# jimonld2000/AudioDenoiser

Measured on AMD Instinct MI355X. Metric: spectrogram frames/sec (forward), 513x256 fp32, higher is better.
Workload: dtype f32; 1 GPU; BASELINE configs[1]: batch=64 synthetic 513x256 fp32 spectrograms on one MI355X, full U-Net forward + per-clip perceptual loss; batch_per_gpu=64, global_batch=64, freq_bins=513, frames=256, parallelism=clips sharded over 1 rank(s), weights replicated, no data-path collective, lib_digest=616623384a0f

## Files before the change

audiodenoiser_amd/csrc/adn_internal.h:

```cpp
#pragma once
#include <hip/hip_runtime.h>
#include <atomic>
#include <cstddef>
#include <cstdint>
#include <type_traits>

namespace adn {

template <typename T> constexpr int ACT_BLOCK = 32 / (int)sizeof(T);
template <typename T>
__host__ __device__ __forceinline__ long act_off(int C, long HW, long pix, int c)
{
    constexpr int B = ACT_BLOCK<T>;
    (void)C;
    return ((long)(c / B) * HW + pix) * B + (c % B);
}

#ifdef __HIPCC__
typedef float f32x2 __attribute__((ext_vector_type(2)));
typedef float f32x4 __attribute__((ext_vector_type(4)));
typedef float f32x16 __attribute__((ext_vector_type(16)));
typedef _Float16 f16x2 __attribute__((ext_vector_type(2)));
typedef _Float16 f16x4 __attribute__((ext_vector_type(4)));
typedef _Float16 f16x8 __attribute__((ext_vector_type(8)));
// ... 185 lines not shown
struct ConvGeom {
    int TH;
    int BN;
    int KC;
};
ConvGeom conv_geom(ConvKind kind, int Cout, bool f16);
long conv_mfma_tiles(ConvKind kind, bool f16, ConvArgs &a);

template <auto... KERNELS>
hipError_t lds_opt_in(size_t bytes)
{
    static std::atomic<unsigned long long> done{0};
    int dev = 0;
    if (hipGetDevice(&dev) != hipSuccess) return hipErrorInvalidDevice;
    const unsigned long long bit = 1ull << (dev & 63);
    if (done.load(std::memory_order_acquire) & bit) return hipSuccess;
    for (const void *k : {reinterpret_cast<const void *>(KERNELS)...}) {
        const hipError_t e = hipFuncSetAttribute(k, hipFuncAttributeMaxDynamicSharedMemorySize, (int)bytes);
        if (e != hipSuccess) return e;
    }
    done.fetch_or(bit, std::memory_order_release);
    return hipSuccess;
}
inline int device_cus()
{
    static std::atomic<int> cus{0};
    int c = cus.load(std::memory_order_relaxed);
    if (c == 0) {
        int dev = 0;
        if (hipGetDevice(&dev) != hipSuccess || hipDeviceGetAttribute(&c, hipDeviceAttributeMultiprocessorCount, dev) != hipSuccess || c < 8)
            return 0;
        c &= ~7;
        cus.store(c, std::memory_order_relaxed);
    }
    return c;
}

hipError_t launch_conv_mfma(ConvKind kind, const ConvArgs &a, bool f16, hipStream_t st);
hipError_t launch_conv_reduce(ConvKind kind, const ConvArgs &a, bool f16, hipStream_t st);
hipError_t launch_convt_reduce(const float *partial, const float *bias, float *out, int ksplit, int N, int Ho, int Wo, int Cout,
                               hipStream_t st);
constexpr int WINO_BN = 32;
hipError_t launch_wino_conv(ConvKind kind, const ConvArgs &a, hipStream_t st);
long wino_tiles(ConvArgs &a);
bool wino4_applicable(ConvKind kind, const ConvArgs &a, bool force);
long wino4_workgroups(const ConvArgs &a);
hipError_t launch_wino4_conv(ConvKind kind, const ConvArgs &a, hipStream_t st);

struct Wino3sGeom {
    int tilesY, tilesX;
    long rows;
    size_t v_bytes, m_bytes;
    long gemm_grid;
};
enum SplitTile { SPLIT_BN128 = 0, SPLIT_BN256 = 1, SPLIT_BN256W8 = 2 };
inline int split_tile_bn(SplitTile t) { return t == SPLIT_BN128 ? 128 : 256; }
bool wino3s_applicable(ConvKind kind, const ConvArgs &a);
Wino3sGeom wino3s_geom(const ConvArgs &a);
hipError_t launch_wino3s_conv(ConvKind kind, const ConvArgs &a, float *V, float *M, SplitTile tile, hipStream_t st);
hipError_t launch_wino_gemm(const float *V, const void *U, float *M, long rows, int Cin, int Cout, SplitTile tile, hipStream_t st);

bool conv16_applicable(ConvKind kind, const ConvArgs &a);
hipError_t launch_conv16(ConvKind kind, const ConvArgs &a, bool resident, hipStream_t st);

bool convt16_applicable(const ConvArgs &a);
hipError_t launch_convt16(const ConvArgs &a, hipStream_t st);

hipError_t launch_conv_first(const float *x, const float *w9x64, const float *bias, void *out, bool f16,
                             int N, int H, int W, int Cin, hipStream_t st);
hipError_t launch_dot_finish(const float *planes, int nplanes, float bias, float *y, long npix, hipStream_t st);
hipError_t launch_conv_out(const void *in, bool f16, const float *w64, float bias, float *out, long npix, long HW,
                           long out_stride, hipStream_t st);
hipError_t launch_nhwc_to_nchw(const void *in, bool f16, float *out, int N, int H, int W, int C, hipStream_t st);

hipError_t launch_stft_mag(const float *audio, int n_clips, long L, int n_fft, int hop, int center, long n_frames,
                           float *out, int rows, long row_stride, long clip_stride, int quantize, hipStream_t st);
constexpr hipError_t ADN_COLD_IN_CAPTURE = hipErrorStreamCaptureUnsupported;
bool stream_is_capturing(hipStream_t st);
hipError_t stft_tables(int n_fft, const float **out, hipStream_t st);
hipError_t loss_tables(hipStream_t st);
hipError_t launch_gl_polar(const float *mag, const float *rnd, int n_clips, int F, int T, void *spec, hipStream_t st);
hipError_t launch_istft_frames(const void *spec, int n_clips, int T, int n_fft, float *buf, hipStream_t st);
hipError_t launch_istft_ola(const float *buf, int n_clips, int T, int n_fft, int hop, float *audio, hipStream_t st);
hipError_t launch_stft_complex(const float *audio, int n_clips, long L, int n_fft, int hop, int T, void *spec,
                               hipStream_t st);
struct DenoiseGeom {
    int T, K, Wd, S, V;
};
bool denoise_geom(int n_frames, int window, int overlap, DenoiseGeom *g);
hipError_t launch_denoise_windows(const void *spec, int n_clips, int F, const DenoiseGeom &g, float *out, hipStream_t st);
hipError_t launch_denoise_stitch(const float *y, int n_clips, int F, const DenoiseGeom &g, int clamp, float *out,
                                 hipStream_t st);
hipError_t launch_denoise_resynth(const float *y, const void *spec, int n_clips, long L, int n_fft, int hop,
                                  const DenoiseGeom &g, float *audio, hipStream_t st);
struct SpectralConsts {
    float smooth, one_minus_smooth, beta, gamma, growth, alpha, one_minus_alpha, gain_floor, bias;
};
hipError_t launch_spectral_gain(const void *spec, int n_clips, int T, int F, const SpectralConsts &k, const float *state_in,
                                float *state_out, float *out, int width, int col0, hipStream_t st);
constexpr int SPECTRAL_MAX_ROWS = 256;
struct SpectralRow {
    int slot, fresh;
};
struct SpectralRows {
    int n;
    SpectralRow row[SPECTRAL_MAX_ROWS];
};
hipError_t launch_spectral_gain_windows(const float *windows, float *y, int n_rows, int n_steps, int F, int W, int col0, int n_cols,
                                        const SpectralConsts &k, float *state, const SpectralRows &rows, hipStream_t st);
struct WpeConsts {
    int K, D, I;
    float loading, rho;
// ... 167 lines not shown
```

audiodenoiser_amd/csrc/unet.hip:

```cpp
#include "adn_host.h"

#include <algorithm>
#include <cmath>
#include <cstdlib>
#include <cstring>
#include <memory>
#include <vector>

using adn::aligned_to;
using adn::DeviceGuard;
using adn::fail;
using adn::fail_hip;

namespace {

constexpr float BN_EPS = 1e-5f;
constexpr int CH[5] = {64, 128, 256, 512, 1024};

enum LayerKind { CONV3, CONVT };
struct LayerDesc {
    LayerKind kind;
    int level;
    int C0, C1;
    int Cout;
};
constexpr int N_CONV3 = 17, N_CONVT = 4, N_LAYERS = N_CONV3 + N_CONVT;
struct LayerTable {
    LayerDesc v[N_LAYERS];
    int n;
};
constexpr LayerTable make_layers()
{
    LayerTable t{};
    for (int l = 0; l <= 4; ++l) {
        if (l > 0) t.v[t.n++] = LayerDesc{CONV3, l, CH[l - 1], 0, CH[l]};
        t.v[t.n++] = LayerDesc{CONV3, l, CH[l], 0, CH[l]};
    }
    for (int l = 3; l >= 0; --l) {
        t.v[t.n++] = LayerDesc{CONVT, l + 1, CH[l + 1], 0, CH[l]};
        t.v[t.n++] = LayerDesc{CONV3, l, CH[l], CH[l], CH[l]};
        t.v[t.n++] = LayerDesc{CONV3, l, CH[l], 0, CH[l]};
    }
    return t;
}
constexpr LayerTable NET = make_layers();
static_assert(NET.n == N_LAYERS && NET.v[0].Cout == 64 && NET.v[8].C0 == 1024 && NET.v[9].kind == CONVT && NET.v[N_LAYERS - 1].Cout == 64,
              "layer table: 9 layers down to the bottleneck, then 4 x (convT, conv, conv)");
static_assert(6 * (1 + N_CONV3) + 2 * N_CONVT + 2 == ADN_N_WEIGHT_TENSORS, "layer table does not match the weight tensor list");
static_assert(1 + N_LAYERS + 1 == ADN_N_LAUNCHES, "layer table does not match the timing slots");

struct LayerWeights {
    size_t w_off, b_off;
    size_t w4_off;
    size_t w3_off;
    adn::SplitTile w3_tile;
    size_t w16_off;
    size_t braw_off;
    size_t wt_off;
};

}

struct adn_unet {
    int device = 0;
    float *dev = nullptr;
    size_t dev_floats = 0;
    size_t first_w = 0, first_b = 0;
    LayerWeights lw[N_LAYERS] = {};
    size_t out_w = 0;
    size_t zero_off = 0;
    float out_b = 0.f;
    std::vector<float> out_bias;
    int in_ch = 1, n_classes = 1;
    std::vector<hipEvent_t> events;
    int timing_max = 0, timing_count = 0;
    bool f16 = false;
    bool use_wino = true;
    bool use_wino4 = true, force_wino4 = false;
    bool allow_split = false;
    bool convt_split = true;
    int f16_conv = 1;
    int f16_convt = 1;
    bool f16_fuse_first = true;
    bool batch_invariant = false;
    long auto_grid = 192, auto_grid64 = 512;
    int wino_gemm = 1;
    long gemm_grid = 1536;
    int split_bn = -1;
    long convt_wide_grid = 2048;
};

namespace {

void bn_fold(const float *b, const float *gamma, const float *beta, const float *mean, const float *var, int C,
             std::vector<float> &scale, std::vector<float> &bias)
{
    scale.resize(C);
    bias.resize(C);
    for (int c = 0; c < C; ++c) {
        const float s = gamma[c] / std::sqrt(var[c] + BN_EPS);
        scale[c] = s;
        bias[c] = (b[c] - mean[c]) * s + beta[c];
    }
}

template <typename T>
void pack_conv3x3(const float *w , const std::vector<float> &scale, int Cin, int Cout, T *dst)
{
    constexpr int EPV = 16 / sizeof(T);
    const adn::ConvGeom g = adn::conv_geom(adn::CONV3X3_RELU, Cout, sizeof(T) == 2);
    const int BN = g.BN, KC = g.KC, KG = KC / (2 * EPV);
    const int nct = Cout / BN, nchunk = Cin / KC;
    size_t o = 0;
    for (int ct = 0; ct < nct; ++ct)
        for (int ch = 0; ch < nchunk; ++ch)
            for (int tap = 0; tap < 9; ++tap)
                for (int s = 0; s < KG; ++s)
                    for (int h = 0; h < 2; ++h)
                        for (int n = 0; n < BN; ++n) {
                            const int co = ct * BN + n;
                            for (int kk = 0; kk < EPV; ++kk) {
                                const int ci = ch * KC + 2 * EPV * s + EPV * h + kk;
                                dst[o++] = (T)(w[((size_t)co * Cin + ci) * 9 + tap] * scale[co]);
                            }
                        }
}

void pack_conv16(const float *w , const std::vector<float> &scale, int Cin, int Cout, _Float16 *dst)
{
    const int nchunk = Cin / 32;
    for (int co = 0; co < Cout; ++co)
        for (int ci = 0; ci < Cin; ++ci) {
            const int ct = co / 64, j = (co % 64) / 16, c16 = co % 16, ch = ci / 32, g = (ci % 32) / 8, e = ci % 8;
            for (int tap = 0; tap < 9; ++tap)
                dst[(((((size_t)ct * nchunk + ch) * 9 + tap) * 4 + j) * 64 + g * 16 + c16) * 8 + e] =
                    (_Float16)(w[((size_t)co * Cin + ci) * 9 + tap] * scale[co]);
        }
}

void pack_wino3x3(const float *w , const std::vector<float> &scale, int Cin, int Cout, int BN,
                  float *dst)
{
    static const double G[4][3] = {{1, 0, 0}, {0.5, 0.5, 0.5}, {0.5, -0.5, 0.5}, {0, 0, 1}};
    const int nct = Cout / BN, nchunk = Cin / 8;
    for (int co = 0; co < Cout; ++co)
// ... 221 lines not shown
    o += p.part_bytes;
    p.total = o;
    return true;
}

adn::ConvArgs conv_args(const adn_unet *h, const Plan &p, int i, const void *in0, const void *in1, int H1, int W1, void *out, void *pool)
{
    const LayerDesc &d = NET.v[i];
    const LayerWeights &L = h->lw[i];
    const int H = p.H[d.level], W = p.W[d.level];
    adn::ConvArgs a = geom_args(d, h->f16, h->use_wino, p.N, H, W);
    a.s0 = adn::ConvSrc{in0, H, W, d.C0, 0, 0};
    if (in1) {
        const int dy = H - H1, dx = W - W1;
        a.s1 = adn::ConvSrc{in1, H1, W1, d.C1, dy / 2, dx / 2};
    } else {
        a.s1 = adn::ConvSrc{in0, 0, 0, 0, 0, 0};
    }
    a.wpk = h->dev + L.w_off;
    a.wpk4 = (h->use_wino && h->use_wino4 && L.w4_off) ? h->dev + L.w4_off : (h->f16 && L.w16_off) ? h->dev + L.w16_off : nullptr;
    a.bias = h->dev + L.b_off;
    a.out = out;
    a.pool = pool;
    return a;
}

adn::ConvArgs convt_args(const adn_unet *h, const Plan &p, int i, const void *in, void *out)
{
    const LayerDesc &d = NET.v[i];
    const int H = p.H[d.level], W = p.W[d.level];
    adn::ConvArgs a = geom_args(d, h->f16, false, p.N, H, W);
    a.s0 = adn::ConvSrc{in, H, W, d.C0, 0, 0};
    a.s1 = adn::ConvSrc{in, 0, 0, 0, 0, 0};
    a.wpk = h->dev + h->lw[i].w_off;
    a.bias = h->dev + h->lw[i].b_off;
    a.out = out;
    a.split = h->convt_split ? 1 : 0;
    return a;
}


enum Conv3Kernel {
    DIRECT,
    CONV16,
    WINO2,
    WINO4,
    WINO3S
};
struct WinoScratch {
    const void *U = nullptr;
    adn::SplitTile tile = adn::SPLIT_BN128;
    float *V = nullptr, *M = nullptr;
    size_t v_bytes = 0, m_bytes = 0;
};
struct Conv3Choice {
    Conv3Kernel kernel;
    int ksplit;
    bool fuse_first;
    bool fuse_out;
};

Conv3Choice choose_conv3(const adn_unet *h, adn::ConvKind kind, const adn::ConvArgs &a, bool first = false, bool tail = false,
                         const WinoScratch &sc = WinoScratch())
{
    Conv3Choice c{DIRECT, 1, false, false};
    if (h->f16) {
        const bool c16 = a.wpk4 && adn::conv16_applicable(kind, a);
        c.fuse_out = tail && a.nct == 1;
        if (first && h->f16_fuse_first && c16) {
            c.kernel = CONV16;
            c.fuse_first = true;
            return c;
        }
        if (a.wpk4 && !h->batch_invariant && !c.fuse_out)
            c.ksplit = adn::conv16_ksplit(adn::conv_workgroups(a), a.nchunk, (size_t)a.N * a.H * a.W * a.Cout);
        if (c.ksplit == 1 && c16) c.kernel = CONV16;
        return c;
    }
    if (!h->use_wino) return c;
    c.kernel = WINO2;
    c.fuse_out = tail && a.nct == 2;
    auto done = [&]() {
        c.fuse_first = first && c.kernel == WINO2 && c.ksplit == 1;
        return c;
    };
    const bool can_split = !c.fuse_out;
    const bool f4_ok = a.wpk4 && adn::wino4_applicable(kind, a, h->force_wino4);
    const long g2 = adn::conv_workgroups(a);
    if (h->allow_split && can_split) {
        c.ksplit = adn::wino_ksplit(g2, a.nchunk);
        if (c.ksplit == 1 && f4_ok) c.kernel = WINO4;
        return done();
    }
    const bool automatic = !h->batch_invariant && !h->force_wino4;
    const long thr = a.Cout <= 64 ? h->auto_grid64 : h->auto_grid;
    const long g4 = f4_ok ? adn::wino4_workgroups(a) : 0;
    if (h->wino_gemm && sc.U && !c.fuse_out && !first && adn::wino3s_applicable(kind, a)) {
        const adn::Wino3sGeom g3 = adn::wino3s_geom(a);
        const bool fits = g3.v_bytes <= sc.v_bytes && g3.m_bytes <= sc.m_bytes;
        const bool pinned = h->batch_invariant && !h->force_wino4;
        if (fits && (h->wino_gemm == 2 || pinned || (automatic && g3.gemm_grid >= h->gemm_grid))) {
            c.kernel = WINO3S;
            return c;
        }
    }
    if (f4_ok && (!automatic || g4 >= thr)) {
        c.kernel = WINO4;
        return done();
    }
    if (automatic && can_split) c.ksplit = adn::wino_ksplit(g2, a.nchunk);
    if (automatic && can_split && f4_ok) {
        const int ks4 = adn::wino4_ksplit(g4, a.nchunk);
        if (ks4 > 1) {
            const double out_mb = (double)a.N * a.H * a.W * a.Cout * 4.0 * 1e-6;
            auto reduce_us = [&](int ks) { return ks > 1 ? 4.0 + (ks + 1) * out_mb / 8.0 : 0.0; };
            const double t4 = 12.0 + 2.79 * (a.nchunk / ks4) * (double)((g4 * ks4 + 255) / 256) + reduce_us(ks4);
            const double t2 = 8.0 + 2.06 * (a.nchunk / c.ksplit) * (double)((g2 * c.ksplit + 511) / 512) + reduce_us(c.ksplit);
            if (t4 < t2) {
                c.kernel = WINO4;
                c.ksplit = ks4;
            }
        }
    }
    return done();
}

hipError_t launch_conv3_kernels(const adn_unet *h, adn::ConvKind kind, const Conv3Choice &c, adn::ConvArgs a, float *partial, hipStream_t st,
                                const WinoScratch &sc)
{
    if (c.fuse_out) kind = adn::CONV3X3_RELU_DOT;
    switch (c.kernel) {
    case WINO3S:
        a.wpk = sc.U;
        return adn::launch_wino3s_conv(kind, a, sc.V, sc.M, sc.tile, st);
    case CONV16:
        a.wpk = a.wpk4;
        a.nchunk0 = a.s0.C / 32;
        a.nchunk = (a.s0.C + a.s1.C) / 32;
        if (c.fuse_first) a.nchunk0 = a.nchunk = 2;
        return adn::launch_conv16(kind, a, c.fuse_first || (a.s0.C + a.s1.C == 64 && a.Cout == 64), st);
    case DIRECT:
        if (c.ksplit > 1) {
            adn::ConvArgs sl = a;
            sl.ksplit = c.ksplit;
            sl.out = partial;
            sl.pool = nullptr;
            hipError_t e = adn::launch_conv_mfma(adn::CONV3X3_RELU, sl, true, st);
            if (e != hipSuccess) return e;
            a.ksplit = c.ksplit;
            a.partial = partial;
            return adn::launch_conv_reduce(kind, a, true, st);
        }
        return adn::launch_conv_mfma(kind, a, h->f16, st);
    case WINO4:
        a.wpk = a.wpk4;
        [[fallthrough]];
    case WINO2:
        a.ksplit = c.ksplit;
        a.partial = partial;
        return c.kernel == WINO4 ? adn::launch_wino4_conv(kind, a, st) : adn::launch_wino_conv(kind, a, st);
    }
    return hipErrorInvalidValue;
}

inline int hip_status(hipError_t e, const char *what)
{
    return e == hipSuccess ? ADN_OK : fail_hip(e, what);
}

int check_part(int layer, int ks, size_t out_floats, size_t part_bytes)
{
    if (ks <= 1 || (size_t)ks * out_floats * sizeof(float) <= part_bytes) return ADN_OK;
    const LayerDesc &d = NET.v[layer];
    return fail(ADN_ERR_WORKSPACE, "adn_unet_forward: layer " + std::to_string(layer) + " (" + (d.kind == CONVT ? "transposed convolution" : "3x3 convolution") +
                " at level " + std::to_string(d.level) + ", " + std::to_string(d.C0 + d.C1) + " -> " + std::to_string(d.Cout) + " channels): " +
                std::to_string(ks) + " K-split copies of " + std::to_string(out_floats * sizeof(float)) + " bytes do not fit the " +
                std::to_string(part_bytes) + " bytes the workspace plan reserves for them");
}

int launch_conv3(const adn_unet *h, int layer, adn::ConvKind kind, const Conv3Choice &c, adn::ConvArgs a, float *partial, size_t part_bytes,
                 hipStream_t st, const WinoScratch &sc = WinoScratch())
{
    if (int rc = check_part(layer, c.ksplit, (size_t)a.N * a.H * a.W * a.Cout, part_bytes)) return rc;
    return hip_status(launch_conv3_kernels(h, kind, c, a, partial, st, sc), "launch_conv3");
}

struct ConvTChoice {
// ... 37 lines not shown
    return adn::launch_conv_mfma(adn::CONVT2X2, a, h->f16, st);
}

int launch_convt(const adn_unet *h, int layer, const ConvTChoice &c, const adn::ConvArgs &a, float *partial, size_t part_bytes, hipStream_t st)
{
    if (int rc = check_part(layer, c.ksplit, (size_t)a.N * (2 * a.H) * (2 * a.W) * a.Cout, part_bytes)) return rc;
    return hip_status(launch_convt_kernels(h, h->lw[layer], c, a, partial, st), "launch_convt");
}


int forward_impl(adn_unet *h, const float *x, float *y, int N, int F, int T, void *workspace, size_t ws_bytes,
                 float *const *taps, hipStream_t st)
{
    if (!h || !x || !y) return fail(ADN_ERR_INVALID, "adn_unet_forward: null handle/x/y");
    Plan p;
    if (!make_plan(N, F, T, h->f16, p)) return fail(ADN_ERR_INVALID, "adn_unet_forward: need N>=1, F,T>=16 and F*T<2^27");
    if (!workspace || ws_bytes < p.total)
        return fail(ADN_ERR_WORKSPACE, "adn_unet_forward: workspace too small (see adn_unet_workspace_bytes)");
    if (!aligned_to(workspace, 16)) return fail(ADN_ERR_INVALID, "adn_unet_forward: workspace must be 16-byte aligned");
    if (!aligned_to(x, 4) || !aligned_to(y, 4)) return fail(ADN_ERR_INVALID, "adn_unet_forward: x and y must be 4-byte aligned");
    DeviceGuard guard(h->device);
    if (guard.err != hipSuccess) return fail_hip(guard.err, "hipSetDevice");

    char *ws = static_cast<char *>(workspace);
    void *tA = ws + p.tA, *tB = ws + p.tB;
    float *part = reinterpret_cast<float *>(ws + p.part);
    const bool f16 = h->f16;
    const bool timed = h->timing_max > 0 && h->timing_count < h->timing_max && !taps;
    hipEvent_t *ev = timed ? h->events.data() + (size_t)h->timing_count * (ADN_N_LAUNCHES + 1) : nullptr;
    int evi = 0;
#define ADN_MARK()                                          \
    do {                                                    \
        if (timed) ADN_HIP(hipEventRecord(ev[evi++], st));  \
    } while (0)

    auto export_tap = [&](int idx, const void *buf, int layer) -> hipError_t {
        if (!taps || !taps[idx]) return hipSuccess;
        const LayerDesc &d = NET.v[layer];
        return adn::launch_nhwc_to_nchw(buf, f16, taps[idx], N, p.H[d.level], p.W[d.level], d.Cout, st);
    };
    int i = 0;
    auto wino_scratch = [&](int li) {
        WinoScratch sc;
        const LayerDesc &d = NET.v[li];
        if (f16 || !h->lw[li].w3_off) return sc;
        const size_t full = (size_t)N * p.H[0] * p.W[0] * 64 * sizeof(float);
        const size_t front = (size_t)N * p.H[d.level] * p.W[d.level] * std::max(std::max(d.C0, d.C1), d.Cout) * sizeof(float);
        if (front >= full) return sc;
        sc.U = h->dev + h->lw[li].w3_off;
        sc.tile = h->lw[li].w3_tile;
        sc.V = reinterpret_cast<float *>(static_cast<char *>(tA) + front);
        sc.M = reinterpret_cast<float *>(static_cast<char *>(tB) + front);
        sc.v_bytes = sc.m_bytes = full - front;
        return sc;
    };

    const void *cur = tA;
    for (int l = 0; l < 4; ++l) {
        void *skip = ws + p.skip[l], *pool = ws + p.pool[l];
        if (l > 0) {
            const WinoScratch sc = wino_scratch(i);
            const adn::ConvArgs a = conv_args(h, p, i++, ws + p.pool[l - 1], nullptr, 0, 0, tA, nullptr);
            ADN_MARK();
            ADN_TRY(launch_conv3(h, i - 1, adn::CONV3X3_RELU, choose_conv3(h, adn::CONV3X3_RELU, a, false, false, sc), a, part, p.part_bytes, st, sc));
        }
        const WinoScratch sc = wino_scratch(i);
        adn::ConvArgs a = conv_args(h, p, i++, cur, nullptr, 0, 0, skip, pool);
        const Conv3Choice c = choose_conv3(h, adn::CONV3X3_RELU_POOL, a, l == 0 && h->in_ch == 1, false, sc);
        if (l == 0) {
            ADN_MARK();
            if (c.fuse_first) {
                a.s0 = adn::ConvSrc{x, p.H[0], p.W[0], 1, 0, 0};
                a.firstw = h->dev + h->first_w;
                a.firstb = h->dev + h->first_b;
            } else {
                ADN_HIP(adn::launch_conv_first(x, h->dev + h->first_w, h->dev + h->first_b, tA, f16, N, p.H[0], p.W[0], h->in_ch, st));
            }
        }
        ADN_MARK();
        ADN_TRY(launch_conv3(h, i - 1, adn::CONV3X3_RELU_POOL, c, a, part, p.part_bytes, st, sc));
        ADN_HIP(export_tap(l, skip, i - 1));
    }
    {
        const WinoScratch sa = wino_scratch(i);
        const adn::ConvArgs a = conv_args(h, p, i++, ws + p.pool[3], nullptr, 0, 0, tA, nullptr);
        ADN_MARK();
        ADN_TRY(launch_conv3(h, i - 1, adn::CONV3X3_RELU, choose_conv3(h, adn::CONV3X3_RELU, a, false, false, sa), a, part, p.part_bytes, st, sa));
        const WinoScratch sb = wino_scratch(i);
        const adn::ConvArgs b = conv_args(h, p, i++, tA, nullptr, 0, 0, tB, nullptr);
        ADN_MARK();
        ADN_TRY(launch_conv3(h, i - 1, adn::CONV3X3_RELU, choose_conv3(h, adn::CONV3X3_RELU, b, false, false, sb), b, part, p.part_bytes, st, sb));
        ADN_HIP(export_tap(4, tB, i - 1));
    }
    void *X = tB, *Y = tA;
    Conv3Choice last{};
    for (int l = 3; l >= 0; --l) {
        const adn::ConvArgs t = convt_args(h, p, i++, X, Y);
        ADN_MARK();
        ADN_TRY(launch_convt(h, i - 1, choose_convt(h, h->lw[i - 1], t), t, part, p.part_bytes, st));
        const WinoScratch sa = wino_scratch(i);
        const adn::ConvArgs a = conv_args(h, p, i++, ws + p.skip[l], Y, 2 * t.H, 2 * t.W, X, nullptr);
        ADN_MARK();
        ADN_TRY(launch_conv3(h, i - 1, adn::CONV3X3_RELU, choose_conv3(h, adn::CONV3X3_RELU, a, false, false, sa), a, part, p.part_bytes, st, sa));
        const WinoScratch sb = wino_scratch(i);
        adn::ConvArgs b = conv_args(h, p, i++, X, nullptr, 0, 0, Y, nullptr);
        last = choose_conv3(h, adn::CONV3X3_RELU, b, false, l == 0 && !taps && h->n_classes == 1, sb);
// ... 16 lines not shown
            ADN_HIP(adn::launch_conv_out(X, f16, h->dev + h->out_w + (size_t)64 * k, h->out_bias[k], y + (size_t)k * F * T,
                                         (long)N * F * T, (long)F * T, (long)h->n_classes * F * T, st));
    ADN_MARK();
    if (timed) {
        if (evi != ADN_N_LAUNCHES + 1) return fail(ADN_ERR_INVALID, "internal: launch count mismatch");
        ++h->timing_count;
    }
#undef ADN_MARK
    if (taps && taps[9])
        ADN_HIP(hipMemcpyAsync(taps[9], y, (size_t)N * h->n_classes * F * T * sizeof(float), hipMemcpyDeviceToDevice, st));
    return ADN_OK;
}


int check_create_args(adn_unet **handle, int device, const float *const *t, int n_tensors, int dtype, int in_channels, int num_classes)
{
    if (!handle || !t) return fail(ADN_ERR_INVALID, "adn_unet_create: null argument");
    if (in_channels < 1 || in_channels > 64 || num_classes < 1 || num_classes > 64)
        return fail(ADN_ERR_INVALID, "adn_unet_create_general: need 1 <= in_channels <= 64 and 1 <= num_classes <= 64");
    if (dtype != ADN_DTYPE_F32 && dtype != ADN_DTYPE_F16) return fail(ADN_ERR_INVALID, "adn_unet_create: dtype must be ADN_DTYPE_F32 or ADN_DTYPE_F16");
    if (n_tensors != ADN_N_WEIGHT_TENSORS) return fail(ADN_ERR_INVALID, "adn_unet_create: expected 118 tensors");
    for (int i = 0; i < n_tensors; ++i)
        if (!t[i]) return fail(ADN_ERR_INVALID, "adn_unet_create: null tensor pointer");
    int ndev = 0;
    if (hipGetDeviceCount(&ndev) != hipSuccess || ndev <= 0) return fail(ADN_ERR_NO_DEVICE, "no HIP device visible");
    if (device < 0 || device >= ndev) return fail(ADN_ERR_INVALID, "adn_unet_create: bad device index");
    return ADN_OK;
}

int check_device_arch(int device)
{
    hipDeviceProp_t prop;
    ADN_HIP(hipGetDeviceProperties(&prop, device));
    if (std::strncmp(prop.gcnArchName, "gfx950", 6) != 0)
        return fail(ADN_ERR_NO_DEVICE, std::string("libadn is built for gfx950 only, device is ") + prop.gcnArchName);
    return ADN_OK;
}

void read_switches(adn_unet &h)
{
    if (const char *algo = std::getenv("ADN_CONV_ALGO"))
        h.use_wino = std::strcmp(algo, "direct") != 0;
    if (h.f16) h.use_wino = false;
    if (const char *sk = std::getenv("ADN_WINO_SPLITK")) h.allow_split = std::atoi(sk) != 0;
    if (const char *cs = std::getenv("ADN_CONVT_SPLIT")) h.convt_split = std::atoi(cs) != 0;
    if (const char *bi = std::getenv("ADN_BATCH_INVARIANT")) h.batch_invariant = std::atoi(bi) != 0;
    if (const char *ff = std::getenv("ADN_F16_FIRST")) h.f16_fuse_first = std::atoi(ff) != 0;
    if (const char *fc = std::getenv("ADN_F16_CONV")) h.f16_conv = std::atoi(fc) == 32 ? 0 : 1;
    if (const char *ft = std::getenv("ADN_F16_CONVT")) h.f16_convt = std::strcmp(ft, "dma") == 0 ? 0 : 1;
    if (const char *ag = std::getenv("ADN_AUTO_GRID")) h.auto_grid = std::atol(ag);
    if (const char *ag = std::getenv("ADN_AUTO_GRID64")) h.auto_grid64 = std::atol(ag);
    if (h.f16) h.convt_split = false;
    if (const char *wg = std::getenv("ADN_WINO_GEMM")) h.wino_gemm = std::atoi(wg) == 2 ? 2 : std::atoi(wg) != 0;
    if (const char *sb = std::getenv("ADN_SPLIT_BN"))
        h.split_bn = !std::strcmp(sb, "128") ? adn::SPLIT_BN128 : !std::strcmp(sb, "256") ? adn::SPLIT_BN256 : !std::strcmp(sb, "256w8") ? adn::SPLIT_BN256W8 : -2;
    if (const char *wt = std::getenv("ADN_WINO_TILE")) {
        h.use_wino4 = std::atoi(wt) != 2;
        h.force_wino4 = std::atoi(wt) == 4;
    }
}

adn::SplitTile split_tile(const adn_unet &h, const LayerDesc &d)
{
    if ((d.kind == CONVT ? 4 * d.Cout : d.Cout) % 256) return adn::SPLIT_BN128;
    if (h.split_bn >= 0) return static_cast<adn::SplitTile>(h.split_bn);
    return d.kind == CONVT && d.Cout < 128 ? adn::SPLIT_BN128 : adn::SPLIT_BN256;
}

void pack_weights(adn_unet &h, const float *const *t, std::vector<float> &host)
{
    auto reserve = [&](size_t n) {
        const size_t at = host.size();
        host.resize(at + ((n + 63) & ~size_t(63)), 0.f);
        return at;
    };
    auto halfs = [&](size_t off) { return reinterpret_cast<_Float16 *>(host.data() + off); };
    std::vector<float> scale, bias;
    bn_fold(t[1], t[2], t[3], t[4], t[5], 64, scale, bias);
    h.first_w = reserve((size_t)h.in_ch * 9 * 64);
    for (int ci = 0; ci < h.in_ch; ++ci)
        for (int tap = 0; tap < 9; ++tap)
            for (int co = 0; co < 64; ++co)
                host[h.first_w + ((size_t)ci * 9 + tap) * 64 + co] = t[0][((size_t)co * h.in_ch + ci) * 9 + tap] * scale[co];
    h.first_b = reserve(64);
    std::memcpy(host.data() + h.first_b, bias.data(), sizeof(float) * 64);
    int ti = 6;
    for (int i = 0; i < N_LAYERS; ++i) {
        const LayerDesc &d = NET.v[i];
        LayerWeights &L = h.lw[i];
        const int Cin = d.C0 + d.C1, Cout = d.Cout;
        const size_t n16 = ((size_t)(d.kind == CONVT ? 4 : 9) * Cin * Cout + 1) / 2;
        if (d.kind == CONVT) {
            if (h.f16) {
                L.w_off = reserve(n16);
                pack_convt<_Float16>(t[ti], Cin, Cout, halfs(L.w_off));
                if (h.f16_convt != 0 && Cin % 128 == 0 && Cout % 64 == 0) {
                    L.w16_off = reserve(n16);
                    pack_convt16(t[ti], Cin, Cout, halfs(L.w16_off));
                    L.braw_off = reserve(Cout);
                    std::memcpy(host.data() + L.braw_off, t[ti + 1], sizeof(float) * Cout);
                }
            } else if (h.convt_split) {
                L.w_off = reserve(3 * n16);
                pack_convt_split(t[ti], Cin, Cout, 128, reinterpret_cast<uint16_t *>(host.data() + L.w_off));
                L.w3_tile = split_tile(h, d);
                if (L.w3_tile != adn::SPLIT_BN128) {
                    L.wt_off = reserve(3 * n16);
                    pack_convt_split(t[ti], Cin, Cout, adn::split_tile_bn(L.w3_tile), reinterpret_cast<uint16_t *>(host.data() + L.wt_off));
                }
                L.braw_off = reserve(Cout);
                std::memcpy(host.data() + L.braw_off, t[ti + 1], sizeof(float) * Cout);
            } else {
                L.w_off = reserve((size_t)4 * Cin * Cout);
                pack_convt<float>(t[ti], Cin, Cout, host.data() + L.w_off);
            }
            L.b_off = reserve((size_t)4 * Cout);
            for (int col = 0; col < 4 * Cout; ++col) {
                int ij, c;
                adn::convt_column(col, Cout, ij, c);
                host[L.b_off + col] = t[ti + 1][c];
            }
            ti += 2;
            continue;
        }
        bn_fold(t[ti + 1], t[ti + 2], t[ti + 3], t[ti + 4], t[ti + 5], Cout, scale, bias);
        if (h.f16 && h.f16_conv != 0 && Cin % 32 == 0 && Cout % 64 == 0) {
            L.w16_off = reserve(n16);
            pack_conv16(t[ti], scale, Cin, Cout, halfs(L.w16_off));
        }
        if (h.use_wino) {
            L.w_off = reserve((size_t)16 * Cin * Cout);
            pack_wino3x3(t[ti], scale, Cin, Cout, adn::WINO_BN, host.data() + L.w_off);
            if (h.use_wino4) {
                L.w4_off = reserve((size_t)36 * Cin * Cout);
                pack_wino4_3x3(t[ti], scale, Cin, Cout, host.data() + L.w4_off);
                if (h.wino_gemm && d.level >= 3 && Cin >= 512 && Cin % 16 == 0 && Cout % 128 == 0) {
                    L.w3_off = reserve((size_t)36 * Cin * Cout * 3 / 2);
                    L.w3_tile = split_tile(h, d);
                    pack_wino4_split(t[ti], scale, Cin, Cout, adn::split_tile_bn(L.w3_tile), reinterpret_cast<uint16_t *>(host.data() + L.w3_off));
                }
            }
        } else if (h.f16) {
            L.w_off = reserve(n16);
            pack_conv3x3<_Float16>(t[ti], scale, Cin, Cout, halfs(L.w_off));
        } else {
            L.w_off = reserve((size_t)9 * Cin * Cout);
            pack_conv3x3<float>(t[ti], scale, Cin, Cout, host.data() + L.w_off);
        }
        L.b_off = reserve(Cout);
        std::memcpy(host.data() + L.b_off, bias.data(), sizeof(float) * Cout);
        ti += 6;
    }
    h.zero_off = reserve(4 * 512);
    h.out_w = reserve((size_t)64 * h.n_classes);
    std::memcpy(host.data() + h.out_w, t[ti], sizeof(float) * 64 * h.n_classes);
    h.out_bias.assign(t[ti + 1], t[ti + 1] + h.n_classes);
    h.out_b = t[ti + 1][0];
}

struct UnetDeleter {
    void operator()(adn_unet *h) const
    {
        {
            DeviceGuard guard(h->device);
            for (hipEvent_t e : h->events) (void)hipEventDestroy(e);
            if (h->dev) (void)hipFree(h->dev);
        }
        delete h;
    }
};

}

extern "C" {

int adn_unet_create(adn_unet **handle, int device, const float *const *t, int n_tensors)
{
    return adn_unet_create_ex(handle, device, t, n_tensors, ADN_DTYPE_F32);
}

int adn_unet_create_ex(adn_unet **handle, int device, const float *const *t, int n_tensors, int dtype)
{
    return adn_unet_create_general(handle, device, t, n_tensors, dtype, 1, 1);
}

int adn_unet_channels(const adn_unet *h, int *in_channels, int *num_classes)
{
    if (!h || !in_channels || !num_classes) return fail(ADN_ERR_INVALID, "adn_unet_channels: null argument");
    *in_channels = h->in_ch;
    *num_classes = h->n_classes;
    return ADN_OK;
}

int adn_unet_set_batch_invariant(adn_unet *h, int on)
{
    if (!h) return fail(ADN_ERR_INVALID, "adn_unet_set_batch_invariant: null handle");
    h->batch_invariant = on != 0;
    return ADN_OK;
}

int adn_unet_create_general(adn_unet **handle, int device, const float *const *t, int n_tensors, int dtype, int in_channels,
                            int num_classes)
{
    if (int rc = check_create_args(handle, device, t, n_tensors, dtype, in_channels, num_classes)) return rc;
    DeviceGuard guard(device);
    if (guard.err != hipSuccess) return fail_hip(guard.err, "hipSetDevice");
    if (int rc = check_device_arch(device)) return rc;

    std::unique_ptr<adn_unet, UnetDeleter> h(new adn_unet());
    h->device = device;
    h->in_ch = in_channels;
    h->n_classes = num_classes;
    h->f16 = dtype == ADN_DTYPE_F16;
    read_switches(*h);
    if (h->split_bn < -1) return fail(ADN_ERR_INVALID, "adn_unet_create: ADN_SPLIT_BN must be 128, 256 or 256w8");
    std::vector<float> host;
    pack_weights(*h, t, host);
    h->dev_floats = host.size();
    hipError_t e = hipMalloc(&h->dev, host.size() * sizeof(float));
    if (e != hipSuccess) return fail_hip(e, "hipMalloc(weights)");
    e = hipMemcpy(h->dev, host.data(), host.size() * sizeof(float), hipMemcpyHostToDevice);
    if (e != hipSuccess) return fail_hip(e, "hipMemcpy(weights)");
    *handle = h.release();
    return ADN_OK;
}

int adn_unet_set_timing(adn_unet *h, int max_forwards)
{
    if (!h || max_forwards < 0 || max_forwards > 4096) return fail(ADN_ERR_INVALID, "adn_unet_set_timing: bad argument");
    DeviceGuard guard(h->device);
    if (guard.err != hipSuccess) return fail_hip(guard.err, "hipSetDevice");
    for (hipEvent_t e : h->events) (void)hipEventDestroy(e);
    h->events.clear();
    h->timing_max = 0;
    h->timing_count = 0;
    h->events.resize((size_t)max_forwards * (ADN_N_LAUNCHES + 1));
    for (size_t i = 0; i < h->events.size(); ++i) ADN_HIP(hipEventCreate(&h->events[i]));
    h->timing_max = max_forwards;
    return ADN_OK;
}

int adn_unet_get_timing(adn_unet *h, int index, float *ms)
{
    if (!h || !ms || index < 0 || index >= h->timing_count) return fail(ADN_ERR_INVALID, "adn_unet_get_timing: no such forward");
    DeviceGuard guard(h->device);
    if (guard.err != hipSuccess) return fail_hip(guard.err, "hipSetDevice");
    hipEvent_t *ev = h->events.data() + (size_t)index * (ADN_N_LAUNCHES + 1);
    ADN_HIP(hipEventSynchronize(ev[ADN_N_LAUNCHES]));
    for (int k = 0; k < ADN_N_LAUNCHES; ++k) ADN_HIP(hipEventElapsedTime(&ms[k], ev[k], ev[k + 1]));
    return ADN_OK;
}

int adn_unet_destroy(adn_unet *h)
{
    if (h) UnetDeleter()(h);
    return ADN_OK;
}

int adn_unet_workspace_bytes(const adn_unet *h, int N, int F, int T, size_t *bytes)
{
    if (!bytes) return fail(ADN_ERR_INVALID, "adn_unet_workspace_bytes: null");
    Plan p;
    if (!make_plan(N, F, T, h ? h->f16 : false, p)) return fail(ADN_ERR_INVALID, "adn_unet_workspace_bytes: need N>=1, F,T>=16 and F*T<2^27");
    *bytes = p.total;
    return ADN_OK;
}

int adn_unet_forward(adn_unet *h, const float *x, float *y, int N, int F, int T, void *workspace,
// ... 13 lines not shown
```

audiodenoiser_amd/csrc/wino3s_kernels.hip:

```cpp
#include "adn_internal.h"

namespace adn {

namespace {

constexpr int NT = 256;

__global__ __launch_bounds__(NT) void wino3s_input_kernel(const ConvArgs p, float *__restrict__ V, int tilesY, int tilesX, long rows)
{
    const long id = (long)blockIdx.x * NT + threadIdx.x;
    const long row = id >> 1;
    const int half = (int)(id & 1), cb = blockIdx.y;
    if (row >= rows) return;
    const int tx = (int)(row % tilesX);
    const long r2 = row / tilesX;
    const int ty = (int)(r2 % tilesY), n = (int)(r2 / tilesY);
    const bool second = cb >= p.s0.C / 8;
    const ConvSrc &s = second ? p.s1 : p.s0;
    const int cbl = second ? cb - p.s0.C / 8 : cb;
    const float *src = static_cast<const float *>(s.ptr) + ((size_t)n * (s.C / 8) + cbl) * ((size_t)s.H * s.W * 8) + half * 4;
    const int y0 = 4 * ty - 1 - s.offY, x0 = 4 * tx - 1 - s.offX;
    f32x4 d[6][6];
#pragma unroll
    for (int a = 0; a < 6; ++a)
#pragma unroll
        for (int b = 0; b < 6; ++b) {
            const int y = y0 + a, x = x0 + b;
            d[a][b] = (y >= 0 && y < s.H && x >= 0 && x < s.W) ? *reinterpret_cast<const f32x4 *>(src + ((size_t)y * s.W + x) * 8)
                                                                : f32x4{0.f, 0.f, 0.f, 0.f};
        }
#pragma unroll
    for (int a = 0; a < 6; ++a) bt6(d[a][0], d[a][1], d[a][2], d[a][3], d[a][4], d[a][5]);
#pragma unroll
    for (int b = 0; b < 6; ++b) bt6(d[0][b], d[1][b], d[2][b], d[3][b], d[4][b], d[5][b]);
    const int ncb = (p.s0.C + p.s1.C) / 8;
    float *vp = V + ((size_t)cb * rows + row) * 8 + half * 4;
    const size_t pstr = (size_t)ncb * rows * 8;
#pragma unroll
    for (int i = 0; i < 6; ++i)
#pragma unroll
        for (int j = 0; j < 6; ++j) *reinterpret_cast<f32x4 *>(vp + (size_t)(6 * i + j) * pstr) = d[i][j];
}

template <bool POOL>
__global__ __launch_bounds__(NT) void wino3s_output_kernel(const ConvArgs p, const float *__restrict__ M, int tilesY, int tilesX,
                                                           long rows)
{
    const long id = (long)blockIdx.x * NT + threadIdx.x;
    const long row = id >> 1;
    const int half = (int)(id & 1), cb = blockIdx.y;
    if (row >= rows) return;
    const int tx = (int)(row % tilesX);
    const long r2 = row / tilesX;
    const int ty = (int)(r2 % tilesY), n = (int)(r2 / tilesY);
    const float *mp = M + ((size_t)cb * rows + row) * 8 + half * 4;
    const size_t pstr = (size_t)(p.Cout / 8) * rows * 8;
    f32x4 w[4][6];
#pragma unroll
    for (int j = 0; j < 6; ++j) {
        f32x4 m[6];
#pragma unroll
        for (int i = 0; i < 6; ++i) m[i] = *reinterpret_cast<const f32x4 *>(mp + (size_t)(6 * i + j) * pstr);
        at6(m[0], m[1], m[2], m[3], m[4], m[5], w[0][j], w[1][j], w[2][j], w[3][j]);
    }
    const f32x4 bias = *reinterpret_cast<const f32x4 *>(p.bias + cb * 8 + half * 4);
    const f32x4 zero = {0.f, 0.f, 0.f, 0.f};
    f32x4 y[4][4];
#pragma unroll
    for (int a = 0; a < 4; ++a) {
        at6(w[a][0], w[a][1], w[a][2], w[a][3], w[a][4], w[a][5], y[a][0], y[a][1], y[a][2], y[a][3]);
#pragma unroll
        for (int b = 0; b < 4; ++b) y[a][b] = __builtin_elementwise_maximum(y[a][b] + bias, zero);
    }
    float *ob = static_cast<float *>(p.out) + ((size_t)n * (p.Cout / 8) + cb) * ((size_t)p.H * p.W * 8) + half * 4;
#pragma unroll
    for (int a = 0; a < 4; ++a)
#pragma unroll
        for (int b = 0; b < 4; ++b) {
            const int gy = 4 * ty + a, gx = 4 * tx + b;
            if (gy < p.H && gx < p.W) *reinterpret_cast<f32x4 *>(ob + ((size_t)gy * p.W + gx) * 8) = y[a][b];
        }
    if constexpr (POOL) {
        const int Hp = p.H >> 1, Wp = p.W >> 1;
        float *pb = static_cast<float *>(p.pool) + ((size_t)n * (p.Cout / 8) + cb) * ((size_t)Hp * Wp * 8) + half * 4;
#pragma unroll
        for (int a = 0; a < 2; ++a)
#pragma unroll
            for (int b = 0; b < 2; ++b) {
                const int py = 2 * ty + a, px = 2 * tx + b;
                const f32x4 mx = __builtin_elementwise_maximum(__builtin_elementwise_maximum(y[2 * a][2 * b], y[2 * a][2 * b + 1]),
                                                               __builtin_elementwise_maximum(y[2 * a + 1][2 * b], y[2 * a + 1][2 * b + 1]));
                if (py < Hp && px < Wp) *reinterpret_cast<f32x4 *>(pb + ((size_t)py * Wp + px) * 8) = mx;
            }
    }
}

}

bool wino3s_applicable(ConvKind kind, const ConvArgs &a)
{
    if (kind != CONV3X3_RELU && kind != CONV3X3_RELU_POOL) return false;
    if (kind == CONV3X3_RELU_POOL && !a.pool) return false;
    const int Cin = a.s0.C + a.s1.C;
    if (a.firstw || a.ksplit > 1 || Cin < 16 || (Cin & 15) || (a.s0.C & 7) || a.Cout < 128 || (a.Cout & 127)) return false;
    return a.N >= 1 && a.H >= 1 && a.W >= 1 && wino3s_geom(a).rows < (1L << 25);
}

Wino3sGeom wino3s_geom(const ConvArgs &a)
{
    Wino3sGeom g{};
    g.tilesY = (a.H + 3) / 4;
    g.tilesX = (a.W + 3) / 4;
    g.rows = (long)a.N * g.tilesY * g.tilesX;
    g.v_bytes = (size_t)36 * g.rows * (a.s0.C + a.s1.C) * sizeof(float);
    g.m_bytes = (size_t)36 * g.rows * a.Cout * sizeof(float);
    g.gemm_grid = 36 * ((g.rows + 127) / 128) * (a.Cout / 128);
    return g;
}

hipError_t launch_wino3s_conv(ConvKind kind, const ConvArgs &a, float *V, float *M, SplitTile tile, hipStream_t st)
{
    if (!wino3s_applicable(kind, a) || !V || !M || !a.wpk || !a.bias || !a.out) return hipErrorInvalidValue;
    const Wino3sGeom g = wino3s_geom(a);
    const long bx = (2 * g.rows + NT - 1) / NT;
    const int Cin = a.s0.C + a.s1.C;
    hipLaunchKernelGGL(wino3s_input_kernel, dim3((unsigned)bx, (unsigned)(Cin / 8)), dim3(NT), 0, st, a, V, g.tilesY, g.tilesX, g.rows);
    hipError_t e = hipGetLastError();
    if (e != hipSuccess) return e;
    e = launch_wino_gemm(V, a.wpk, M, g.rows, Cin, a.Cout, tile, st);
    if (e != hipSuccess) return e;
    if (kind == CONV3X3_RELU_POOL)
        hipLaunchKernelGGL(wino3s_output_kernel<true>, dim3((unsigned)bx, (unsigned)(a.Cout / 8)), dim3(NT), 0, st, a, M, g.tilesY,
                           g.tilesX, g.rows);
    else
        hipLaunchKernelGGL(wino3s_output_kernel<false>, dim3((unsigned)bx, (unsigned)(a.Cout / 8)), dim3(NT), 0, st, a, M, g.tilesY,
                           g.tilesX, g.rows);
    return hipGetLastError();
}

}
```

Baseline: 525,400 frames/s.

## Slice three-stage Winograd conv by tile rows and extend it to more layers

Adds row-slicing to the three-stage Winograd path (input transform, GEMM, output transform), so a layer whose V/M scratch does not fit the available room can run in up to four sequential slices. Uses this to enable the three-stage path by default on two more layers (down4.conv1 and up2.conv1), with a separate, higher grid threshold for those layers, and adds a per-layer table plus an env override. The aim is to replace the direct or wino4 kernels on larger mid-level layers with the GEMM-based path, at the cost of extra launches per slice, repeated weight reads, and extra scratch traffic.

```diff
diff --git a/audiodenoiser_amd/csrc/adn_internal.h b/audiodenoiser_amd/csrc/adn_internal.h
--- a/audiodenoiser_amd/csrc/adn_internal.h
+++ b/audiodenoiser_amd/csrc/adn_internal.h
@@ -261,12 +261,15 @@
     long rows;
     size_t v_bytes, m_bytes;
     long gemm_grid;
+    int slices;
+    long slice_rows;
 };
 enum SplitTile { SPLIT_BN128 = 0, SPLIT_BN256 = 1, SPLIT_BN256W8 = 2 };
 inline int split_tile_bn(SplitTile t) { return t == SPLIT_BN128 ? 128 : 256; }
 bool wino3s_applicable(ConvKind kind, const ConvArgs &a);
 Wino3sGeom wino3s_geom(const ConvArgs &a);
-hipError_t launch_wino3s_conv(ConvKind kind, const ConvArgs &a, float *V, float *M, SplitTile tile, hipStream_t st);
+bool wino3s_slice(const ConvArgs &a, size_t room_v, size_t room_m, int max_slices, int min_slices, Wino3sGeom &g);
+hipError_t launch_wino3s_conv(ConvKind kind, const ConvArgs &a, float *V, float *M, SplitTile tile, hipStream_t st, long slice_rows = 0);
 hipError_t launch_wino_gemm(const float *V, const void *U, float *M, long rows, int Cin, int Cout, SplitTile tile, hipStream_t st);
 
 bool conv16_applicable(ConvKind kind, const ConvArgs &a);
diff --git a/audiodenoiser_amd/csrc/unet.hip b/audiodenoiser_amd/csrc/unet.hip
--- a/audiodenoiser_amd/csrc/unet.hip
+++ b/audiodenoiser_amd/csrc/unet.hip
@@ -5,6 +5,7 @@
 #include <cstdlib>
 #include <cstring>
 #include <memory>
+#include <string>
 #include <vector>
 
 using adn::aligned_to;
@@ -48,6 +49,44 @@
               "layer table: 9 layers down to the bottleneck, then 4 x (convT, conv, conv)");
 static_assert(6 * (1 + N_CONV3) + 2 * N_CONVT + 2 == ADN_N_WEIGHT_TENSORS, "layer table does not match the weight tensor list");
 static_assert(1 + N_LAYERS + 1 == ADN_N_LAUNCHES, "layer table does not match the timing slots");
+
+constexpr const char *LAYER_NAMES[N_LAYERS] = {
+    "down1.conv2", "down2.conv1", "down2.conv2", "down3.conv1", "down3.conv2", "down4.conv1", "down4.conv2", "bottleneck.conv1", "bottleneck.conv2",
+    "up1.convT", "up1.conv1", "up1.conv2", "up2.convT", "up2.conv1", "up2.conv2", "up3.convT", "up3.conv1", "up3.conv2", "up4.convT", "up4.conv1", "up4.conv2"};
+
+constexpr int WINO3S_MAX_SLICES = 4;
+struct Wino3sEntry {
+    int layer;
+    int max_slices;
+    bool by_default;
+    bool f4_only;
+};
+constexpr Wino3sEntry WINO3S_TABLE[] = {
+    {6, 1, true, false},
+    {7, 1, true, false},
+    {8, 1, true, false},
+    {10, 1, true, false},
+    {11, 1, true, false},
+    {4, WINO3S_MAX_SLICES, false, true},
+    {5, WINO3S_MAX_SLICES, true, true},
+    {13, WINO3S_MAX_SLICES, true, true},
+    {14, WINO3S_MAX_SLICES, false, true},
+};
+constexpr const Wino3sEntry *wino3s_entry(int li)
+{
+    for (const Wino3sEntry &e : WINO3S_TABLE)
+        if (e.layer == li) return &e;
+    return nullptr;
+}
+constexpr bool wino3s_table_ok()
+{
+    for (const Wino3sEntry &e : WINO3S_TABLE) {
+        const LayerDesc &d = NET.v[e.layer];
+        if (d.kind != CONV3 || (d.C0 + d.C1) % 16 || d.Cout % 128 || e.max_slices < 1 || e.max_slices > WINO3S_MAX_SLICES) return false;
+    }
+    return true;
+}
+static_assert(wino3s_table_ok(), "three-stage table: 3x3 layers with whole 16-channel chunks and 128-column tiles");
 
 struct LayerWeights {
     size_t w_off, b_off;
@@ -85,12 +124,27 @@
     bool batch_invariant = false;
     long auto_grid = 192, auto_grid64 = 512;
     int wino_gemm = 1;
-    long gemm_grid = 1536;
+    long gemm_grid = 1536, gemm_grid_later = 3456;
+    unsigned wino_layers = 0;
+    bool bad_layers = false;
+    int wino_slices = 1;
     int split_bn = -1;
     long convt_wide_grid = 2048;
 };
 
 namespace {
+
+int wino3s_layer(const adn_unet &h, int li)
+{
+    const Wino3sEntry *e = wino3s_entry(li);
+    return e && (e->by_default || (h.wino_layers >> li & 1)) ? e->max_slices : 0;
+}
+
+bool wino3s_f4_only(const adn_unet &h, int li)
+{
+    const Wino3sEntry *e = wino3s_entry(li);
+    return e && e->f4_only && !(h.wino_layers >> li & 1);
+}
 
 void bn_fold(const float *b, const float *gamma, const float *beta, const float *mean, const float *var, int C,
              std::vector<float> &scale, std::vector<float> &bias)
@@ -418,18 +472,22 @@
     adn::SplitTile tile = adn::SPLIT_BN128;
     float *V = nullptr, *M = nullptr;
     size_t v_bytes = 0, m_bytes = 0;
+    int max_slices = 1;
+    bool f4_only = false;
+    long min_grid = 0;
 };
 struct Conv3Choice {
     Conv3Kernel kernel;
     int ksplit;
     bool fuse_first;
     bool fuse_out;
+    long slice_rows;
 };
 
 Conv3Choice choose_conv3(const adn_unet *h, adn::ConvKind kind, const adn::ConvArgs &a, bool first = false, bool tail = false,
                          const WinoScratch &sc = WinoScratch())
 {
-    Conv3Choice c{DIRECT, 1, false, false};
+    Conv3Choice c{DIRECT, 1, false, false, 0};
     if (h->f16) {
         const bool c16 = a.wpk4 && adn::conv16_applicable(kind, a);
         c.fuse_out = tail && a.nct == 1;
@@ -461,12 +519,13 @@
     const bool automatic = !h->batch_invariant && !h->force_wino4;
     const long thr = a.Cout <= 64 ? h->auto_grid64 : h->auto_grid;
     const long g4 = f4_ok ? adn::wino4_workgroups(a) : 0;
-    if (h->wino_gemm && sc.U && !c.fuse_out && !first && adn::wino3s_applicable(kind, a)) {
-        const adn::Wino3sGeom g3 = adn::wino3s_geom(a);
-        const bool fits = g3.v_bytes <= sc.v_bytes && g3.m_bytes <= sc.m_bytes;
+    if (h->wino_gemm && sc.U && !c.fuse_out && !first && (!sc.f4_only || f4_ok) && adn::wino3s_applicable(kind, a)) {
+        adn::Wino3sGeom g3 = adn::wino3s_geom(a);
+        const bool fits = adn::wino3s_slice(a, sc.v_bytes, sc.m_bytes, sc.max_slices, h->wino_slices, g3);
         const bool pinned = h->batch_invariant && !h->force_wino4;
-        if (fits && (h->wino_gemm == 2 || pinned || (automatic && g3.gemm_grid >= h->gemm_grid))) {
+        if (fits && (h->wino_gemm == 2 || pinned || (automatic && g3.gemm_grid / g3.slices >= sc.min_grid))) {
             c.kernel = WINO3S;
+            c.slice_rows = g3.slices > 1 ? g3.slice_rows : 0;
             return c;
         }
     }
@@ -498,7 +557,7 @@
     switch (c.kernel) {
     case WINO3S:
         a.wpk = sc.U;
-        return adn::launch_wino3s_conv(kind, a, sc.V, sc.M, sc.tile, st);
+        return adn::launch_wino3s_conv(kind, a, sc.V, sc.M, sc.tile, st, c.slice_rows);
     case CONV16:
         a.wpk = a.wpk4;
         a.nchunk0 = a.s0.C / 32;
@@ -642,6 +701,9 @@
         sc.V = reinterpret_cast<float *>(static_cast<char *>(tA) + front);
         sc.M = reinterpret_cast<float *>(static_cast<char *>(tB) + front);
         sc.v_bytes = sc.m_bytes = full - front;
+        sc.max_slices = wino3s_layer(*h, li);
+        sc.f4_only = wino3s_f4_only(*h, li);
+        sc.min_grid = wino3s_entry(li)->f4_only ? h->gemm_grid_later : h->gemm_grid;
         return sc;
     };
 
@@ -764,6 +826,20 @@
     if (const char *ag = std::getenv("ADN_AUTO_GRID64")) h.auto_grid64 = std::atol(ag);
     if (h.f16) h.convt_split = false;
     if (const char *wg = std::getenv("ADN_WINO_GEMM")) h.wino_gemm = std::atoi(wg) == 2 ? 2 : std::atoi(wg) != 0;
+    if (const char *ws = std::getenv("ADN_WINO_SLICES")) h.wino_slices = std::min(std::max(std::atoi(ws), 1), 64);
+    if (const char *wl = std::getenv("ADN_WINO_GEMM_LAYERS")) {
+        const std::string list(wl);
+        for (size_t at = 0; at <= list.size();) {
+            const size_t end = std::min(list.find(',', at), list.size());
+            const std::string name = list.substr(at, end - at);
+            int li = -1;
+            for (int i = 0; i < N_LAYERS; ++i)
+                if (name == LAYER_NAMES[i] && wino3s_entry(i)) li = i;
+            if (li >= 0) h.wino_layers |= 1u << li;
+            else if (!name.empty()) h.bad_layers = true;
+            at = end + 1;
+        }
+    }
     if (const char *sb = std::getenv("ADN_SPLIT_BN"))
         h.split_bn = !std::strcmp(sb, "128") ? adn::SPLIT_BN128 : !std::strcmp(sb, "256") ? adn::SPLIT_BN256 : !std::strcmp(sb, "256w8") ? adn::SPLIT_BN256W8 : -2;
     if (const char *wt = std::getenv("ADN_WINO_TILE")) {
@@ -846,7 +922,7 @@
             if (h.use_wino4) {
                 L.w4_off = reserve((size_t)36 * Cin * Cout);
                 pack_wino4_3x3(t[ti], scale, Cin, Cout, host.data() + L.w4_off);
-                if (h.wino_gemm && d.level >= 3 && Cin >= 512 && Cin % 16 == 0 && Cout % 128 == 0) {
+                if (h.wino_gemm && wino3s_layer(h, i)) {
                     L.w3_off = reserve((size_t)36 * Cin * Cout * 3 / 2);
                     L.w3_tile = split_tile(h, d);
                     pack_wino4_split(t[ti], scale, Cin, Cout, adn::split_tile_bn(L.w3_tile), reinterpret_cast<uint16_t *>(host.data() + L.w3_off));
@@ -926,6 +1002,7 @@
     h->f16 = dtype == ADN_DTYPE_F16;
     read_switches(*h);
     if (h->split_bn < -1) return fail(ADN_ERR_INVALID, "adn_unet_create: ADN_SPLIT_BN must be 128, 256 or 256w8");
+    if (h->bad_layers) return fail(ADN_ERR_INVALID, "adn_unet_create: ADN_WINO_GEMM_LAYERS names a layer the three-stage table does not hold");
     std::vector<float> host;
     pack_weights(*h, t, host);
     h->dev_floats = host.size();
diff --git a/audiodenoiser_amd/csrc/wino3s_kernels.hip b/audiodenoiser_amd/csrc/wino3s_kernels.hip
--- a/audiodenoiser_amd/csrc/wino3s_kernels.hip
+++ b/audiodenoiser_amd/csrc/wino3s_kernels.hip
@@ -1,4 +1,6 @@
 #include "adn_internal.h"
+
+#include <algorithm>
 
 namespace adn {
 
@@ -6,14 +8,16 @@
 
 constexpr int NT = 256;
 
-__global__ __launch_bounds__(NT) void wino3s_input_kernel(const ConvArgs p, float *__restrict__ V, int tilesY, int tilesX, long rows)
+__global__ __launch_bounds__(NT) void wino3s_input_kernel(const ConvArgs p, float *__restrict__ V, int tilesY, int tilesX, long rows,
+                                                          long row0)
 {
     const long id = (long)blockIdx.x * NT + threadIdx.x;
     const long row = id >> 1;
     const int half = (int)(id & 1), cb = blockIdx.y;
     if (row >= rows) return;
-    const int tx = (int)(row % tilesX);
-    const long r2 = row / tilesX;
+    const long grow = row0 + row;
+    const int tx = (int)(grow % tilesX);
+    const long r2 = grow / tilesX;
     const int ty = (int)(r2 % tilesY), n = (int)(r2 / tilesY);
     const bool second = cb >= p.s0.C / 8;
     const ConvSrc &s = second ? p.s1 : p.s0;
@@ -44,14 +48,15 @@
 
 template <bool POOL>
 __global__ __launch_bounds__(NT) void wino3s_output_kernel(const ConvArgs p, const float *__restrict__ M, int tilesY, int tilesX,
-                                                           long rows)
+                                                           long rows, long row0)
 {
     const long id = (long)blockIdx.x * NT + threadIdx.x;
     const long row = id >> 1;
     const int half = (int)(id & 1), cb = blockIdx.y;
     if (row >= rows) return;
-    const int tx = (int)(row % tilesX);
-    const long r2 = row / tilesX;
+    const long grow = row0 + row;
+    const int tx = (int)(grow % tilesX);
+    const long r2 = grow / tilesX;
     const int ty = (int)(r2 % tilesY), n = (int)(r2 / tilesY);
     const float *mp = M + ((size_t)cb * rows + row) * 8 + half * 4;
     const size_t pstr = (size_t)(p.Cout / 8) * rows * 8;
@@ -115,27 +120,52 @@
     g.v_bytes = (size_t)36 * g.rows * (a.s0.C + a.s1.C) * sizeof(float);
     g.m_bytes = (size_t)36 * g.rows * a.Cout * sizeof(float);
     g.gemm_grid = 36 * ((g.rows + 127) / 128) * (a.Cout / 128);
+    g.slices = 1;
+    g.slice_rows = g.rows;
     return g;
 }
 
-hipError_t launch_wino3s_conv(ConvKind kind, const ConvArgs &a, float *V, float *M, SplitTile tile, hipStream_t st)
+bool wino3s_slice(const ConvArgs &a, size_t room_v, size_t room_m, int max_slices, int min_slices, Wino3sGeom &g)
+{
+    const size_t row_v = (size_t)36 * (a.s0.C + a.s1.C) * sizeof(float), row_m = (size_t)36 * a.Cout * sizeof(float);
+    const long cap1 = (long)std::min(room_v / a.N / row_v, room_m / a.N / row_m), per_clip = (long)g.tilesY * g.tilesX;
+    if (cap1 < 1) return false;
+    const long need = (per_clip + cap1 - 1) / cap1;
+    if (need > max_slices) return false;
+    const long S = std::max(need, (long)min_slices);
+    if (S == 1) return true;
+    long len = (g.rows + S - 1) / S;
+    const long cap = (long)std::min(room_v / row_v, room_m / row_m), len128 = (len + 127) / 128 * 128;
+    if (len128 <= cap && (g.rows + len128 - 1) / len128 == (g.rows + len - 1) / len) len = len128;
+    g.slice_rows = len;
+    g.slices = (int)((g.rows + len - 1) / len);
+    return true;
+}
+
+hipError_t launch_wino3s_conv(ConvKind kind, const ConvArgs &a, float *V, float *M, SplitTile tile, hipStream_t st, long slice_rows)
 {
     if (!wino3s_applicable(kind, a) || !V || !M || !a.wpk || !a.bias || !a.out) return hipErrorInvalidValue;
     const Wino3sGeom g = wino3s_geom(a);
-    const long bx = (2 * g.rows + NT - 1) / NT;
     const int Cin = a.s0.C + a.s1.C;
-    hipLaunchKernelGGL(wino3s_input_kernel, dim3((unsigned)bx, (unsigned)(Cin / 8)), dim3(NT), 0, st, a, V, g.tilesY, g.tilesX, g.rows);
-    hipError_t e = hipGetLastError();
-    if (e != hipSuccess) return e;
-    e = launch_wino_gemm(V, a.wpk, M, g.rows, Cin, a.Cout, tile, st);
-    if (e != hipSuccess) return e;
-    if (kind == CONV3X3_RELU_POOL)
-        hipLaunchKernelGGL(wino3s_output_kernel<true>, dim3((unsigned)bx, (unsigned)(a.Cout / 8)), dim3(NT), 0, st, a, M, g.tilesY,
-                           g.tilesX, g.rows);
-    else
-        hipLaunchKernelGGL(wino3s_output_kernel<false>, dim3((unsigned)bx, (unsigned)(a.Cout / 8)), dim3(NT), 0, st, a, M, g.tilesY,
-                           g.tilesX, g.rows);
-    return hipGetLastError();
+    if (slice_rows < 1 || slice_rows > g.rows) slice_rows = g.rows;
+    for (long row0 = 0; row0 < g.rows; row0 += slice_rows) {
+        const long rows = std::min(slice_rows, g.rows - row0);
+        const long bx = (2 * rows + NT - 1) / NT;
+        hipLaunchKernelGGL(wino3s_input_kernel, dim3((unsigned)bx, (unsigned)(Cin / 8)), dim3(NT), 0, st, a, V, g.tilesY, g.tilesX, rows, row0);
+        hipError_t e = hipGetLastError();
+        if (e != hipSuccess) return e;
+        e = launch_wino_gemm(V, a.wpk, M, rows, Cin, a.Cout, tile, st);
+        if (e != hipSuccess) return e;
+        if (kind == CONV3X3_RELU_POOL)
+            hipLaunchKernelGGL(wino3s_output_kernel<true>, dim3((unsigned)bx, (unsigned)(a.Cout / 8)), dim3(NT), 0, st, a, M, g.tilesY,
+                               g.tilesX, rows, row0);
+        else
+            hipLaunchKernelGGL(wino3s_output_kernel<false>, dim3((unsigned)bx, (unsigned)(a.Cout / 8)), dim3(NT), 0, st, a, M, g.tilesY,
+                               g.tilesX, rows, row0);
+        e = hipGetLastError();
+        if (e != hipSuccess) return e;
+    }
+    return hipSuccess;
 }
 
 }
```

New measurement: 524,400 frames/s. About the same (-0.2%).
